# tpatten/squirrel_motion_planner

Hardware: AMD Instinct MI355X
Metric: collision-checked samples/sec + time-to-first-feasible-path, 8-DoF, 5 cm octomap (higher is better)
Workload: dtype f64

## Files before the change

### squirrel_motion_planner_amd/csrc/smp_kernels.hip

```cpp
#include <hip/hip_runtime.h>

#include <vector>

#include "smp_collide.h"
#include "smp_math.h"
#include "smp_plan.h"
#include "smp_types.h"

extern "C" __device__ __attribute__((const)) unsigned long long __ockl_wfred_min_u64(unsigned long long);
extern "C" __device__ __attribute__((const)) unsigned long long __ockl_wfred_max_u64(unsigned long long);

namespace smp {

constexpr int CHECK_CT = 32;

__shared__ RobotDev g_rb;
__shared__ MapCfg g_mc;
__shared__ WideStash g_wk;

__device__ __forceinline__ void stage_model(const RobotDev* rb, const MapCfg* mc, RobotDev* rbl, MapCfg* mcl) {
  static_assert(sizeof(RobotDev) % 8 == 0 && sizeof(MapCfg) % 4 == 0, "staging granularity");
  for (int i = threadIdx.x; i < (int)(sizeof(RobotDev) / 8); i += BLOCK)
    reinterpret_cast<uint64_t*>(rbl)[i] = reinterpret_cast<const uint64_t*>(rb)[i];
  for (int i = threadIdx.x; i < (int)(sizeof(MapCfg) / 4); i += BLOCK)
// ... 122 lines not shown
    }
  __syncthreads();
  for (int wd = 0; wd < (nsph + 31) / 32; ++wd) {
    uint32_t m = cand[wd];
    while (m) {
      const int s = wd * 32 + __builtin_ctz(m);
      m &= m - 1;
      const int c = rb->sph_clink[s];
      if (lm[c]) continue;
      const bool hit = wave_sphere_map(sc, wc[s], rb->sph_r[s], lane);
      __syncthreads();
      if (hit && lane == 0) lm[c] = 1;
      __syncthreads();
    }
  }
  for (int c = lane; c < rb->n_clink; c += 64) link_map[c] = (uint8_t)lm[c];
  for (int p = lane; p < rb->n_pairs; p += 64) {
    const int a = rb->pair_a[p], b = rb->pair_b[p];
    bool hit = false;
    if (rb->cl_prim[a] >= 0 || rb->cl_prim[b] >= 0) {
      const int pr = rb->cl_prim[a] >= 0 ? rb->cl_prim[a] : rb->cl_prim[b], sl = rb->cl_prim[a] >= 0 ? b : a;
      for (int s = rb->cl_sph0[sl]; s < rb->cl_sph0[sl] + rb->cl_nsph[sl] && !hit; ++s)
        hit = sphere_prim(rb->prim_type[pr], &rb->prim_h[pr * 3], pwl[pr], wc[s], rb->sph_r[s]);
      pair_self[p] = hit ? 1 : 0;
      continue;
    }
    for (int sa = rb->cl_sph0[a]; sa < rb->cl_sph0[a] + rb->cl_nsph[a] && !hit; ++sa)
      for (int sb = rb->cl_sph0[b]; sb < rb->cl_sph0[b] + rb->cl_nsph[b]; ++sb) {
        const double rs = rb->sph_r[sa] + rb->sph_r[sb];
        const double ex = wc[sa][0] - wc[sb][0], ey = wc[sa][1] - wc[sb][1], ez = wc[sa][2] - wc[sb][2];
        if (ex * ex + ey * ey + ez * ez <= rs * rs) { hit = true; break; }
      }
    pair_self[p] = hit ? 1 : 0;
  }
}

void launch_collisions(hipStream_t st, const RobotDev* rb, SceneDev sc, const MapCfg* mc, const double* q, int map,
                       uint8_t* link_map, uint8_t* pair_self) {
  hipLaunchKernelGGL(collisions_kernel, dim3(1), dim3(64), 0, st, rb, sc, mc, q, map, link_map, pair_self);
}

__global__ void sincos_kernel(const double* x, int n, double* s, double* c) {
  int i = blockIdx.x * blockDim.x + threadIdx.x;
  if (i < n) psincos(x[i], s + i, c + i);
}

__global__ void u01_kernel(unsigned long long seed, unsigned query, const uint32_t* ctr, int n, double* out) {
  int i = blockIdx.x * blockDim.x + threadIdx.x;
  if (i < n) out[i] = u01(seed, query, ctr[4 * i], ctr[4 * i + 1], ctr[4 * i + 2], ctr[4 * i + 3]);
}

__global__ void __launch_bounds__(128) fk_kernel(const RobotDev* __restrict__ rb, const double* q, int n, double* frames, double* eez) {
  int i = blockIdx.x * blockDim.x + threadIdx.x;
  if (i >= n) return;
  double qq[NJ];
  for (int j = 0; j < NJ; ++j) qq[j] = q[i * NJ + j];
  Frame B[MAX_BODY];
  body_frames(rb, qq, B);
  for (int b = 0; b < rb->n_body; ++b) {
    for (int k = 0; k < 9; ++k) frames[((size_t)i * rb->n_body + b) * 12 + k] = B[b].R[k];
    for (int k = 0; k < 3; ++k) frames[((size_t)i * rb->n_body + b) * 12 + 9 + k] = B[b].p[k];
  }
  eez[i] = ee_z(rb, qq);
}

__global__ void sqrt_div_kernel(const double* a, const double* b, int n, double* sq, double* dv) {
  int i = blockIdx.x * blockDim.x + threadIdx.x;
  if (i < n) { sq[i] = sqrt(a[i]); dv[i] = a[i] / b[i]; }
}

constexpr int SCAN_K = 20;
constexpr int NEAR_BINS = 256;
constexpr int NEAR_BUF = 128;
#ifndef SMP_NEAR_NBK
#define SMP_NEAR_NBK 16
#endif
constexpr int NEAR_NBK = SMP_NEAR_NBK;
struct ScanLds {
  union {
    struct {
      unsigned long long wlk[BLOCK / 64][SCAN_K], whk[BLOCK / 64][SCAN_K];
      int wli[BLOCK / 64][SCAN_K], whi[BLOCK / 64][SCAN_K];
    };
    struct {
      alignas(16) unsigned hist[NEAR_BINS];
      unsigned long long ck[2][NEAR_BUF];
      int ci[2][NEAR_BUF];
    };
  };
  unsigned long long hmin[BLOCK / 64], hmax[BLOCK / 64];
  int hcnt[2], hblo, hbhi, fast;
  int wtot[BLOCK / 64];
  unsigned long long blo, bhi;
  unsigned long long lk[SCAN_K], hk[SCAN_K];
  int li[SCAN_K], hi[SCAN_K];
  int cnt, take;
  unsigned long long wk[BLOCK / 64];
  int wi[BLOCK / 64];
};
constexpr int MERGE_LS = SCAN_K | 1;
struct MergeLds {
  unsigned kl[2][SCAN_PNEAR][MERGE_LS], kh[2][SCAN_PNEAR][MERGE_LS];
  int id[2][SCAN_PNEAR][MERGE_LS];
  int len[SCAN_P], cnt[SCAN_P], done[SCAN_P], bad[SCAN_P];
  unsigned hv[SCAN_P][3];
  unsigned hn[SCAN_PNEAR][3];
  unsigned long long nk[SCAN_P];
  int ni[SCAN_P];
  int ndone, go[2], steal;
};
__device__ __forceinline__ unsigned long long merge_key(const MergeLds& M, int s, int w, int e) {
  return (unsigned long long)M.kh[s][w][e] << 32 | M.kl[s][w][e];
}
struct JobLds {
#ifdef SMP_NO_SCAN_UNION
  ScanLds scan;
  WideLds T;
#else
  union {
    ScanLds scan;
    WideLds T;
  };
#endif
  double tq[TILE_CT_MAX][NJ];
  double start[MAXE][NJ], step[MAXE][NJ];
  unsigned words[JOB_WORDS];
  uint8_t rmask[JOB_TILES];
  uint8_t rdone[JOB_TILES];
  int emap[MAXE];
  int first[MAXE];
  int E, np1, nslots, ntiles, ct, self, map, seq, steal, hidx, left;
  int skip, sfv, tskip;
  int tgrp[TILE_CT_MAX], tord[TILE_CT_MAX];
  unsigned long long tprof[4];
  int go[2];
};
struct SmpLds {
  double q[64][NJ];
  int ok[64];
  int win;
};
struct SamplerLds {
  QState S;
  SmpLds W;
  double out[NJ];
  long long next;
  int ver, go[2];
};
#ifndef SMP_PLAN_CT
#define SMP_PLAN_CT 8
#endif
constexpr int PLAN_CT = SMP_PLAN_CT;
constexpr int PATCH_K = 32;
struct PlanLds {
  QState S;
  union {
    struct {
      TileLds<PLAN_CT> T;
      double tq[PLAN_CT][NJ];
    } tile;
    JobLds job;
    double seg[MAXE][MAX_PTS][3];
    SmpLds smp;
    SamplerLds smpl;
  } u;
  union {
    struct {
      struct {
        unsigned long long wlk[BLOCK / 64][MAX_NEAR], whk[BLOCK / 64][MAX_NEAR];
        int wli[BLOCK / 64][MAX_NEAR], whi[BLOCK / 64][MAX_NEAR];
        int wtot[BLOCK / 64];
      } nr;
      struct {
        alignas(16) unsigned hist[NEAR_BINS];
        unsigned long long ck[2][NEAR_BUF];
        int ci[2][NEAR_BUF];
        unsigned long long wmin[BLOCK / 64], wmax[BLOCK / 64];
        int wtot[BLOCK / 64];
        int cnt[2], blo, bhi, fast;
      } nh;
    };
    struct {
      ScanLds s;
      MergeLds m;
    } sc;
  };
  double eg_start[MAXE][NJ], eg_target[MAXE][NJ], eg_step[MAXE][NJ], eg_end[MAXE][NJ];
  double eg_base[MAXE][3], eg_cost[MAXE][3];
  double eg_acc[MAXE][3];
  int eg_first[MAXE], eg_need[MAXE], eg_near[MAXE], eg_ptr[MAXE];
  int rw_par[MAXE], rw_next;
  double rw_cost[MAXE][3];
  int tile_e[PLAN_CT], tile_i[PLAN_CT], tile_n;
  int count_slot;
  int job_seq;
  int in_job;
  int go_end;
  int smp_ver, smp_have_sol, smp_hit;
  int smp_pub;
  int spec, spec_nn;
  long long spec_cnt;
  double smp_cbest[3];
  int nk;
  unsigned long long near_blo, near_bhi;
  int lo_i[MAX_NEAR], hi_i[MAX_NEAR];
  double lo_c[MAX_NEAR], hi_c[MAX_NEAR];
  int n_lo, n_hi;
  NodeRef nn, xn, xc, cur, g;
  double xr[NJ], ext[NJ], ox[NJ];
  double en_start[NJ], en_target[NJ];
  int ext_nn, ext_bp, flag, found, nn_id, cnt;
  int reached;
  int n_via, nn_t, tree_expand;
  NodeRef sel;
  double sel_start[NJ], sel_target[NJ];
  double csp[3], best_nv;
  double sol[3];
  double wd[BLOCK / 64];
  unsigned long long wk[BLOCK / 64];
  int wi[BLOCK / 64];
  long long wcount[BLOCK / 64];
  ScoutRec sr;
  PreRec prer;
  int prer_ok;
#ifdef SMP_TRACE
  int trole;
  unsigned tn;
  long long tit;
#endif
  int sp_on, sp_stage, sp_go[2];
  double fnn_d;
  int fnn_id;
#ifdef SMP_SCAN_PROF
  unsigned long long spc_t;
#endif
  int sc_same[MAX_SCOUTS];
  unsigned sc_seen, sc_dead;
  int asked[SCOUT_SLOTS];
  int asked_conn[SCOUT_SLOTS];
  int asked_pre[SCOUT_SLOTS];
  int conn_rec;
  int two_scouts;
  unsigned sc_mod;
  unsigned rw_at0;
  int n_at0;
  int sc_t, sc_rerun;
  int sc_stale_f;
  double sc_hq[MAXE][NJ], sc_hc[MAXE];
  int sc_hp[MAXE];
  int rb_go[2];
  long long sc_k;
  int eg_hit[MAXE];
  int eg_rec[MAXE];
  int rec_grp;
  int rec_all, ev_job;
  double pc_q[2][PATCH_K][NJ];
};

__shared__ PlanLds g_L;

struct Ctx {
  SceneDev sc;
  QueryDev Q;
};

#ifdef SMP_TRACE
#ifndef SMP_TRACE_IT0
#define SMP_TRACE_IT0 3000
#endif
#ifndef SMP_TRACE_IT1
#define SMP_TRACE_IT1 3040
#endif
constexpr unsigned TLOG_CAP = 1u << 18, TLOG_ROLE = TLOG_CAP / 4;
__device__ unsigned long long g_tlog[TLOG_CAP];
__device__ unsigned g_tlog_n[4];
#define TR()                                                                                                  \
  if (threadIdx.x == 0 && g_L.tit >= SMP_TRACE_IT0 && g_L.tit < SMP_TRACE_IT1 && g_L.tn < TLOG_ROLE) {        \
    g_tlog[g_L.trole * TLOG_ROLE + g_L.tn] =                                                                   \
        ((unsigned long long)g_L.trole << 62) | ((unsigned long long)((g_L.tit - SMP_TRACE_IT0) & 0xff) << 54) | \
        ((unsigned long long)(__LINE__ & 0x3fff) << 40) | (wall_clock64() & 0xffffffffffull);                  \
    g_tlog_n[g_L.trole] = ++g_L.tn;                                                                            \
  }
#else
#define TR()
#endif

enum { P_SAMPLE, P_NN, P_EXPAND, P_NEAR, P_CHOOSE, P_REWIRE, P_CONNECT, P_TILES, P_NTILES, P_COSTS, P_VIA, P_NVIA,
       P_TFK, P_TCHAIN, P_TCENTRE, P_TTEST, P_XEXPAND, P_XCHOOSE, P_XREWIRE, P_XCONNECT };
#ifdef SMP_NOCLK
__device__ __forceinline__ unsigned long long pclk() { return 0; }
#else
__device__ __forceinline__ unsigned long long pclk() { return wall_clock64(); }
#endif
#define PROF_BEGIN() unsigned long long _pt = threadIdx.x == 0 ? pclk() : 0
#ifdef SMP_DETAIL_PROF
#define DETAIL_BEGIN(v) const unsigned long long v = threadIdx.x == 0 ? wall_clock64() : 0
#define DETAIL_END(v, k) if (threadIdx.x == 0) g_L.S.prof[k] += wall_clock64() - v
#else
#define DETAIL_BEGIN(v)
#define DETAIL_END(v, k)
#endif
#define PROF_END(k) if (threadIdx.x == 0) { g_L.S.prof[k] += pclk() - _pt; }

__device__ __forceinline__ int lane_id() { return threadIdx.x & 63; }
__device__ __forceinline__ int uni(int v) { return __builtin_amdgcn_readfirstlane(v); }
__device__ __forceinline__ int wave_id() { return threadIdx.x >> 6; }
typedef const double __attribute__((address_space(1)))* gcdptr;
__device__ __forceinline__ gcdptr uni_gptr(const double* p) {
  const unsigned long long v = reinterpret_cast<unsigned long long>(p);
  const unsigned lo = __builtin_amdgcn_readfirstlane((int)(unsigned)v);
  const unsigned hi = __builtin_amdgcn_readfirstlane((int)(unsigned)(v >> 32));
  return (gcdptr)(((unsigned long long)hi << 32) | lo);
}

__device__ __forceinline__ gcdptr uni_g(gcdptr p) {
  const unsigned long long v = reinterpret_cast<unsigned long long>(p);
  const unsigned lo = __builtin_amdgcn_readfirstlane((int)(unsigned)v);
  const unsigned hi = __builtin_amdgcn_readfirstlane((int)(unsigned)(v >> 32));
  return (gcdptr)(((unsigned long long)hi << 32) | lo);
}
__device__ __forceinline__ void tree_cols(gcdptr tq, int cap, gcdptr* c) {
#pragma unroll
  for (int j = 0; j < NJ; ++j) c[j] = uni_g(tq + (size_t)j * (unsigned)cap);
}
__device__ __forceinline__ bool wave_group_live(int first, int end) {
  return __builtin_amdgcn_readfirstlane((int)(first < end)) != 0;
}
__device__ __forceinline__ double ld_col(gcdptr col, unsigned i) {
  return *(gcdptr)((const char __attribute__((address_space(1)))*)col + i * 8u);
}
typedef const float __attribute__((address_space(1)))* gcfptr;
__device__ __forceinline__ float ld_col(gcfptr col, unsigned i) {
  return *(gcfptr)((const char __attribute__((address_space(1)))*)col + i * 4u);
}
template <int K, int NPT, typename P, typename T>
__device__ __forceinline__ void load_round_k(T (*a)[NJ], const P* cols, int b0, int i1, const T* fill) {
#pragma unroll
  for (int u = 0; u < NPT; ++u) {
    if (u < K) {
      const unsigned ii = (unsigned)min(b0 + u * BLOCK, i1 - 1);
#pragma unroll
      for (int j = 0; j < NJ; ++j) a[u][j] = ld_col(cols[j], ii);
    } else {
#pragma unroll
      for (int j = 0; j < NJ; ++j) a[u][j] = fill[j];
    }
  }
}
template <int NPT, typename P, typename T>
__device__ __forceinline__ void load_round(T (*a)[NJ], const P* cols, int b0, int i1, const T* fill) {
  static_assert(NPT == 8, "rounds of 8 nodes per thread");
  const int first = b0 - lane_id();
  const int nl = uni(min(NPT, (i1 - first + BLOCK - 1) / BLOCK));
  if (nl > 4) load_round_k<8, NPT>(a, cols, b0, i1, fill);
  else if (nl > 2) load_round_k<4, NPT>(a, cols, b0, i1, fill);
  else if (nl > 1) load_round_k<2, NPT>(a, cols, b0, i1, fill);
  else load_round_k<1, NPT>(a, cols, b0, i1, fill);
}

__device__ __forceinline__ void st_tree(double* p, double v) { *p = v; }
__device__ __forceinline__ void st_tree(int* p, int v) { *p = v; }
__device__ __forceinline__ void st_tree(float* p, float v) { *p = v; }
__device__ __forceinline__ void st_coord(const TreeDev& T, int cap, int j, int i, double v) {
  st_tree(&T.q[(size_t)j * cap + i], v);
  st_tree(&T.qf[(size_t)j * cap + i], (float)v);
}
__device__ __forceinline__ int xcc_id() { return __builtin_amdgcn_s_getreg((3 << 11) | 20); }
__device__ __forceinline__ bool same8(const double* a, const double* b) {
  bool s = true;
#pragma unroll
  for (int j = 0; j < NJ; ++j) s &= __double_as_longlong(a[j]) == __double_as_longlong(b[j]);
  return s;
}

#ifdef SMP_BOUNDS
__device__ int g_dbg[8];
#define BCHK(id, lim, line, t)                                                                          \
  if ((unsigned)(id) >= (unsigned)(lim)) {                                                             \
    if (atomicCAS(&g_dbg[0], 0, (line)) == 0) { g_dbg[1] = (id); g_dbg[2] = blockIdx.x; g_dbg[3] = (t); g_dbg[4] = (lim); } \
    id = 0;                                                                                            \
  }
#else
#define BCHK(id, lim, line, t)
#endif
#define load_node(C, t, id, o) load_node_at(C, t, id, o, __LINE__)
__device__ __forceinline__ void load_node_at(const Ctx& C, int t, int id, NodeRef* o, int line) {
  const TreeDev& T = C.Q.tr[t];
  const int cap = g_L.S.cap;
  BCHK(id, cap, line, t);
  (void)line;
  for (int j = 0; j < NJ; ++j) o->q[j] = T.q[(size_t)j * cap + id];
  for (int k = 0; k < 3; ++k) o->c[k] = T.cost[(size_t)k * cap + id];
  o->id = id;
  o->parent = T.parent[id];
}

__device__ void insert_node(const Ctx& C, int t, const double* e_start, const double* e_target, const NodeRef& x) {
  QState& S = g_L.S;
  int i = S.n[t];
  if (i >= S.cap || x.id != i) { S.status = -7; S.phase = 2; return; }
  const TreeDev& T = C.Q.tr[t];
  int cap = S.cap;
  for (int j = 0; j < NJ; ++j) {
    st_coord(T, cap, j, i, x.q[j]);
    T.e_start[(size_t)j * cap + i] = e_start[j];
    T.e_target[(size_t)j * cap + i] = e_target[j];
    g_L.pc_q[t][i & (PATCH_K - 1)][j] = x.q[j];
  }
  for (int k = 0; k < 3; ++k) st_tree(&T.cost[(size_t)k * cap + i], x.c[k]);
  st_tree(&T.parent[i], x.parent);
  T.first_child[i] = -1;
  int p = x.parent;
// ... 1245 lines not shown
      if (threadIdx.x == 0) { g_L.n_lo = take_c; g_L.n_hi = take_c; }
      __syncthreads();
      NEAR_COUNT(27);
      continue;
    }
    const double cmin = __longlong_as_double((long long)kmin), cmax = __longlong_as_double((long long)kmax);
    const double scale = cmax > cmin ? (NEAR_BINS * (1.0 - 1e-9)) / (cmax - cmin) : 0.0;
    unsigned bins[NEAR_NBK / 4] = {};
#pragma unroll
    for (int b = 0; b < NEAR_NBK; ++b)
      if (nmask >> b & 1) {
        const int bin = near_bin(key[b], cmin, scale);
        bins[b >> 2] |= (unsigned)bin << (8 * (b & 3));
        atomicAdd(&g_L.nh.hist[bin], 1u);
      }
    __syncthreads();
    NEAR_CLOCK(2);
    if (wave == 0) {
      const uint4 hv = reinterpret_cast<const uint4*>(g_L.nh.hist)[lane];
      const unsigned h0 = hv.x, h1 = hv.y, h2 = hv.z, h3 = hv.w;
      const int inc = wave_incl_scan(h0 + h1 + h2 + h3);
      const int c3 = inc, c2 = c3 - (int)h3, c1 = c2 - (int)h2, c0b = c1 - (int)h1;
      const int e0 = c0b - (int)h0;
      const int flo = c0b >= take_c ? 0 : c1 >= take_c ? 1 : c2 >= take_c ? 2 : c3 >= take_c ? 3 : 4;
      const int Llo = __builtin_ctzll(__ballot(flo < 4));
      const int blo = 4 * Llo + __builtin_amdgcn_readlane(flo, Llo);
      const int cnt_lo = __builtin_amdgcn_readlane(flo == 0 ? c0b : flo == 1 ? c1 : flo == 2 ? c2 : c3, Llo);
      const int lim = tot - take_c;
      const int fhi = c2 <= lim ? 3 : c1 <= lim ? 2 : c0b <= lim ? 1 : e0 <= lim ? 0 : -1;
      const int Lhi = 63 - __builtin_clzll(__ballot(fhi >= 0));
      const int fh = __builtin_amdgcn_readlane(fhi, Lhi);
      const int bhi = 4 * Lhi + fh;
      const int cnt_hi = tot - __builtin_amdgcn_readlane(fhi == 3 ? c2 : fhi == 2 ? c1 : fhi == 1 ? c0b : e0, Lhi);
      if (lane == 0) {
        g_L.nh.blo = blo;
        g_L.nh.bhi = bhi;
        g_L.nh.fast = cnt_lo + prev_lo <= NEAR_BUF && cnt_hi + prev_hi <= NEAR_BUF;
        g_L.nh.cnt[0] = prev_lo;
        g_L.nh.cnt[1] = prev_hi;
      }
    }
    if (threadIdx.x < prev_lo) {
      g_L.nh.ck[0][threadIdx.x] = (unsigned long long)__double_as_longlong(g_L.lo_c[threadIdx.x]);
      g_L.nh.ci[0][threadIdx.x] = g_L.lo_i[threadIdx.x];
    }
    if (threadIdx.x >= 64 && threadIdx.x < 64 + prev_hi) {
      g_L.nh.ck[1][threadIdx.x - 64] = (unsigned long long)__double_as_longlong(g_L.hi_c[threadIdx.x - 64]);
      g_L.nh.ci[1][threadIdx.x - 64] = g_L.hi_i[threadIdx.x - 64];
    }
    __syncthreads();
    NEAR_CLOCK(3);
    if (!uni(g_L.nh.fast)) {
      NEAR_COUNT(26);
      __syncthreads();
      near_set_stream<K, NN>(C, t, q, excl);
      return;
    }
    const int blo = g_L.nh.blo, bhi = g_L.nh.bhi;
#pragma unroll
    for (int g = 0; g < NEAR_NBK; ++g) {
      if (c0 + g * BLOCK + wave * 64 < n) {
        const bool nr = nmask >> g & 1;
        const int bin = bins[g >> 2] >> (8 * (g & 3)) & 255;
        const int i = c0 + g * BLOCK + wave * 64 + lane;
        if (nr && bin <= blo) {
          const int slot = atomicAdd(&g_L.nh.cnt[0], 1);
          g_L.nh.ck[0][slot] = key[g];
          g_L.nh.ci[0][slot] = i;
        }
        if (nr && bin >= bhi) {
          const int slot = atomicAdd(&g_L.nh.cnt[1], 1);
          g_L.nh.ck[1][slot] = key[g];
          g_L.nh.ci[1][slot] = i;
        }
      }
    }
    __syncthreads();
    NEAR_CLOCK(4);
    const int take = min(K, tot_all + tot);
    {
      const int e = threadIdx.x >= 256;
      const int idx = threadIdx.x & 255;
      const int m = g_L.nh.cnt[e];
      const int L = m <= 64 ? 4 : 2;
      const int c = L == 4 ? idx >> 2 : idx >> 1, sl = idx & (L - 1);
      int rank = 0;
      unsigned long long ck = 0;
      int ci = 0;
      if (c < m) {
        ck = g_L.nh.ck[e][c];
        ci = g_L.nh.ci[e][c];
        for (int j = sl; j < m; j += L) {
          const unsigned long long ok = g_L.nh.ck[e][j];
          const int oi = g_L.nh.ci[e][j];
          rank += e == 0 ? ki_less(ok, oi, ck, ci) : ki_less(ck, ci, ok, oi);
        }
      }
      rank += quad_xor1(rank);
      if (L == 4) rank += quad_xor2(rank);
      if (c < m && sl == 0 && rank < take) {
        if (e == 0) { g_L.lo_c[rank] = __longlong_as_double((long long)ck); g_L.lo_i[rank] = ci; }
        else { g_L.hi_c[take - 1 - rank] = __longlong_as_double((long long)ck); g_L.hi_i[take - 1 - rank] = ci; }
      }
    }
    tot_all += tot;
    if (threadIdx.x == 0) { g_L.n_lo = take; g_L.n_hi = take; }
    __syncthreads();
    NEAR_CLOCK(5);
    NEAR_COUNT(27);
  }
  if (threadIdx.x == 0) { g_L.nk = tot_all; g_L.S.near_nodes += n; }
  __syncthreads();
  if (NN) fnn_reduce(nb, nbi);
  TR();
}

template <int K, bool NN>
__device__ __noinline__ void near_set_scan(const Ctx& C, int t, const double* q, int excl) {
  [[clang::always_inline]] near_set<K, NN>(C, t, q, excl, false);
}

__device__ __forceinline__ unsigned rev_mask(const RobotDev* rb) {
  unsigned m = 0;
#pragma unroll
  for (int j = 0; j < NJ; ++j) m |= (rb->rev[j] != 0 ? 1u : 0u) << j;
  return m;
}

__device__ __forceinline__ double readlane_d(double v, int l) {
  const unsigned long long b = (unsigned long long)__double_as_longlong(v);
  const unsigned lo = (unsigned)__builtin_amdgcn_readlane((int)(unsigned)b, l);
  const unsigned hi = (unsigned)__builtin_amdgcn_readlane((int)(unsigned)(b >> 32), l);
  return __longlong_as_double((long long)(((unsigned long long)hi << 32) | lo));
}

__device__ __forceinline__ void seg_terms(unsigned rm, const double* st, const double* stp, int s, double& t, double& r,
                                          double& p) {
  t = 0.0; r = 0.0; p = 0.0;
#pragma unroll
  for (int j = 0; j < NJ; ++j) {
    const double a = st[j] + s * stp[j];
    const double b = st[j] + (s + 1) * stp[j];
    const double d = (b - a) * (b - a);
    t += d * 1.0;
    const bool rv = (rm >> j) & 1u;
    r += rv ? d : 0.0;
    p += rv ? 0.0 : d;
  }
}
__device__ __forceinline__ void seg_norms(unsigned rm, const double* st, const double* stp, int s, double& t, double& r,
                                          double& p) {
  seg_terms(rm, st, stp, s, t, r, p);
  t = sqrt(t); r = sqrt(r); p = sqrt(p);
}

__device__ void edge_costs(const Ctx& C, int E) {
  TR();
  PROF_BEGIN();
  const int np = g_L.S.n_pts;
  const RobotDev* rb = (&g_rb);
  if (threadIdx.x < E * NJ) {
    int e = threadIdx.x / NJ, j = threadIdx.x - e * NJ;
    double st = (g_L.eg_target[e][j] - g_L.eg_start[e][j]) / double(np);
    g_L.eg_step[e][j] = st;
    g_L.eg_end[e][j] = g_L.eg_start[e][j] + np * st;
  }
  __syncthreads();
  const unsigned rm = rev_mask(rb);
  for (int it = threadIdx.x; it < E * np; it += BLOCK) {
    const int e = it / np, s = it - e * np;
    double st[NJ], stp[NJ], t, r, p;
#pragma unroll
    for (int j = 0; j < NJ; ++j) { st[j] = g_L.eg_start[e][j]; stp[j] = g_L.eg_step[e][j]; }
    seg_norms(rm, st, stp, s, t, r, p);
    g_L.u.seg[e][s][0] = t;
    g_L.u.seg[e][s][1] = r;
    g_L.u.seg[e][s][2] = p;
  }
  __syncthreads();
  if (threadIdx.x < E * 3) {
    int e = threadIdx.x / 3, k = threadIdx.x - e * 3;
    double sg[MAX_PTS];
#pragma unroll
    for (int s = 0; s < MAX_PTS; ++s) sg[s] = g_L.u.seg[e][s][k];
    double acc = 0.0;
#pragma unroll
    for (int s = 0; s < MAX_PTS; ++s)
      if (s < np) acc += sg[s];
    g_L.eg_acc[e][k] = acc;
    g_L.eg_cost[e][k] = g_L.eg_base[e][k] + acc;
  }
  __syncthreads();
  PROF_END(P_COSTS);
  TR();
}

__device__ void edge_costs_acc(int E, const double (*acc)[3]) {
  const int np = g_L.S.n_pts;
  if (threadIdx.x < E * NJ) {
    const int e = threadIdx.x / NJ, j = threadIdx.x - e * NJ;
    const double st = (g_L.eg_target[e][j] - g_L.eg_start[e][j]) / double(np);
    g_L.eg_step[e][j] = st;
    g_L.eg_end[e][j] = g_L.eg_start[e][j] + np * st;
  } else if (threadIdx.x >= 256 && threadIdx.x < 256 + E * 3) {
    const int i = threadIdx.x - 256, e = i / 3, k = i - e * 3;
    const double a = acc[e][k];
    g_L.eg_acc[e][k] = a;
    g_L.eg_cost[e][k] = g_L.eg_base[e][k] + a;
  }
  __syncthreads();
}

#define TRACE(C, slot, v) \
  if ((C).Q.trace) __hip_atomic_store(&(C).Q.trace[slot], (int)(v), __ATOMIC_RELAXED, __HIP_MEMORY_SCOPE_SYSTEM)
__device__ __forceinline__ void st_agent(int* p, int v) { __hip_atomic_store(p, v, __ATOMIC_RELAXED, __HIP_MEMORY_SCOPE_AGENT); }
__device__ __forceinline__ void st_agent(unsigned long long* p, unsigned long long v) {
  __hip_atomic_store(p, v, __ATOMIC_RELAXED, __HIP_MEMORY_SCOPE_AGENT);
}
__device__ __forceinline__ int ld_agent(const int* p) { return __hip_atomic_load(p, __ATOMIC_RELAXED, __HIP_MEMORY_SCOPE_AGENT); }
__device__ __forceinline__ unsigned long long ld_agent(const unsigned long long* p) {
  return __hip_atomic_load(p, __ATOMIC_RELAXED, __HIP_MEMORY_SCOPE_AGENT);
}
__device__ __forceinline__ unsigned ld_agent(const unsigned* p) {
  return __hip_atomic_load(p, __ATOMIC_RELAXED, __HIP_MEMORY_SCOPE_AGENT);
}
__device__ __forceinline__ void drain() { asm volatile("s_waitcnt vmcnt(0)" ::: "memory"); }

__device__ __forceinline__ unsigned long long granule(int seq, unsigned w) {
  return ((unsigned long long)(unsigned)seq << 32) | w;
}

__device__ __forceinline__ bool job_tile_skip(const Ctx& C, JobLds& J, int t, int seq) {
  const JobBoard* jb = C.Q.jb;
  const int np1 = uni(J.np1), ne = uni(J.E), ct = uni(J.ct);
  for (int u = threadIdx.x; u < t; u += BLOCK) {
    if (!J.rdone[u]) {
      const unsigned long long v = ld_agent(&jb->res[u]);
      if ((int)(v >> 32) == seq) { J.rmask[u] = (unsigned)v; J.rdone[u] = 1; }
    }
  }
  if (threadIdx.x < ne) J.first[threadIdx.x] = np1;
  __syncthreads();
  for (int u = threadIdx.x; u < t; u += BLOCK) {
    if (!J.rdone[u]) continue;
    unsigned m = J.rmask[u];
    while (m) {
      const int sl = u * ct + __builtin_ctz(m), k = sl / np1;
      m &= m - 1;
      atomicMin(&J.first[k], sl - k * np1);
    }
  }
  __syncthreads();
  if (threadIdx.x < 64) {
    const int lane = threadIdx.x;
    bool fr = false;
    if (J.sfv && lane < ne && (lane + 1) * np1 <= t * ct && J.first[lane] >= np1) {
      fr = true;
      for (int u = (lane * np1) / ct; u <= ((lane + 1) * np1 - 1) / ct; ++u)
        if (!J.rdone[u]) { fr = false; break; }
    }
    const unsigned long long fb = __ballot(fr);
    const int ff = fb ? __builtin_ctzll(fb) : (1 << 30);
    const int base = t * ct, nc = min(ct, J.nslots - base);
    bool live = false;
    if (lane < nc) {
      const int sl = base + lane, k = sl / np1, i = sl - k * np1;
      live = k <= ff && i <= J.first[k];
      J.tgrp[lane] = k;
      J.tord[lane] = live ? i : (1 << 30);
    }
    const unsigned long long lb = __ballot(live);
    if (lane == 0) J.tskip = lb == 0;
  }
  __syncthreads();
  return uni(J.tskip) != 0;
}

struct DirectJob {
  unsigned hdr;
  int ne;
};
__device__ __forceinline__ unsigned job_tile_mask(const Ctx& C, const WideConst& K, JobLds& J, int t,
                                                  unsigned long long* prof = nullptr, int seq = -1,
                                                  const DirectJob* direct = nullptr, bool sync_after = true) {
  int ct, nc, self, map;
  bool sk = false;
  if (direct) {
    const unsigned hdr = direct->hdr;
    const int ne = direct->ne;
    const int np1 = (int)((hdr >> 8) & 255);
    ct = 1 << ((hdr >> 21) & 3);
    const int base = t * ct;
    nc = min(ct, ne * np1 - base);
    self = (int)((hdr >> 16) & 1);
    map = (int)((hdr >> 17) & 1);
    const int c = (int)(threadIdx.x >> 6) / (NWAVE / ct), j = threadIdx.x & 63;
    if (c < nc && j < NJ) {
      const int sl = base + c, k = sl / np1, i = sl - k * np1, wi = 1 + 32 * k + 2 * j;
      const double qs = __hiloint2double((int)J.words[wi + 1], (int)J.words[wi]);
      const double qd = __hiloint2double((int)J.words[wi + 2 * NJ + 1], (int)J.words[wi + 2 * NJ]);
      J.tq[c][j] = qs + i * qd;
    }
    wave_sync();
  } else {
    ct = uni(J.ct);
    const int base = t * ct;
// ... 1062 lines not shown
      if (threadIdx.x < E && g_L.eg_hit[threadIdx.x] >= 0) g_L.eg_first[threadIdx.x] = g_L.eg_hit[threadIdx.x];
      __syncthreads();
    }
    TR();
    return;
  }
  if (threadIdx.x < E) { g_L.eg_first[threadIdx.x] = np1; g_L.eg_ptr[threadIdx.x] = 0; }
  sc_early_send(C, early, epar, E, true);
  __syncthreads();
  for (;;) {
    if (threadIdx.x < 64) {
      const int e = threadIdx.x;
      const bool live = e < E && g_L.eg_need[e] && g_L.eg_first[e] >= np1;
      const int ptr = e < E ? g_L.eg_ptr[e] : np1;
      bool stop = false;
      if (stop_first_valid) {
        const unsigned long long m = __ballot(live);
        if (m) stop = __shfl(ptr, __builtin_ctzll(m)) >= np1;
      }
      const int rem = (live && ptr < np1) ? np1 - ptr : 0;
      int inc = rem;
      for (int off = 1; off < 32; off <<= 1) {
        int v = __shfl_up(inc, off);
        if (e >= off) inc += v;
      }
      const int start = inc - rem;
      const int take = stop ? 0 : max(0, min(rem, PLAN_CT - start));
      for (int i = 0; i < take; ++i) { g_L.tile_e[start + i] = e; g_L.tile_i[start + i] = ptr + i; }
      if (e < E) g_L.eg_ptr[e] = ptr + take;
      const int total = __shfl(inc, 31);
      if (e == 0) g_L.tile_n = stop ? 0 : min(PLAN_CT, total);
    }
    __syncthreads();
    const int nc = uni(g_L.tile_n);
    if (nc == 0) break;
    if (threadIdx.x < nc * NJ) {
      int c = threadIdx.x / NJ, j = threadIdx.x - c * NJ;
      int e = g_L.tile_e[c];
      g_L.u.tile.tq[c][j] = g_L.eg_start[e][j] + g_L.tile_i[c] * g_L.eg_step[e][j];
    }
    __syncthreads();
    PROF_BEGIN();
    local_tile(C, nc);
    PROF_END(P_TILES);
    if (threadIdx.x == 0) {
      g_L.S.prof[pslot] += pclk() - _pt;
      g_L.S.prof[P_NTILES]++;
      g_L.S.prof[pslot + 8] += nc;
    }
  }
  __syncthreads();
  overlap_work(C, ov, ovt);
}

__device__ void overlap_work(const Ctx& C, int ov, int t) {
  ov = uni(ov);
  t = uni(t);
  if (ov == OV_NONE) {
    if (threadIdx.x == 0) g_L.spec = OV_NONE;
    __syncthreads();
    return;
  }
  const long long c0 = ov == OV_NN ? g_L.S.nn_nodes : g_L.S.near_nodes;
  __syncthreads();
  if (ov == OV_NEAR_EXPAND) near_set<20>(C, t, g_L.eg_end[0], g_L.S.n[t], true);
  else if (ov == OV_NEAR_XN) near_set<20>(C, t, g_L.xn.q, g_L.xn.id);
  else {
    const int id = nearest(C, t, g_L.xn.q);
    if (threadIdx.x == 0) g_L.spec_nn = id;
  }
  if (threadIdx.x == 0) {
    long long& cnt = ov == OV_NN ? g_L.S.nn_nodes : g_L.S.near_nodes;
    g_L.spec_cnt = cnt - c0;
    cnt = c0;
    g_L.spec = ov;
  }
  __syncthreads();
}

__device__ __forceinline__ void count_edge(int first) {
  int np1 = g_L.S.n_pts + 1;
  g_L.S.prof[g_L.count_slot] += first >= np1 ? np1 : first + 1;
  if (first >= np1) { g_L.S.checked += np1; g_L.S.valid += np1; }
  else { g_L.S.checked += first + 1; g_L.S.valid += first; }
}

__device__ int count_edges(int E, bool stop_first) {
  if (threadIdx.x < 64) {
    const int e = threadIdx.x, np1 = g_L.S.n_pts + 1;
    const bool need = e < E && g_L.eg_need[e];
    const int f = need ? g_L.eg_first[e] : 0;
    const unsigned long long mfree = __ballot(need && f >= np1);
    const int ev = (stop_first && mfree) ? __builtin_ctzll(mfree) : 64;
    int chk = 0, val = 0;
    if (need && e <= ev) { chk = f >= np1 ? np1 : f + 1; val = f >= np1 ? np1 : f; }
    chk = __ockl_wfred_add_i32(chk); val = __ockl_wfred_add_i32(val);
    if (e == 0) {
      g_L.S.prof[g_L.count_slot] += chk;
      g_L.S.checked += chk;
      g_L.S.valid += val;
      g_L.found = ev < 64 ? ev : -1;
    }
  }
  __syncthreads();
  return uni(g_L.found);
}

__device__ __forceinline__ bool step_towards_m(unsigned rm, const double* nn, double* x, double f) {
  double ed[NJ], srev = 0.0, spr = 0.0;
#pragma unroll
  for (int j = 0; j < NJ; ++j) {
    const bool rv = (rm >> j) & 1u;
    ed[j] = x[j] - nn[j];
    const double d = ed[j] * ed[j];
    srev += rv ? d : 0.0;
    spr += rv ? 0.0 : d;
  }
  const double lrev = sqrt(srev), lpr = sqrt(spr);
  const bool rev_done = lrev < 0.001, pr_done = lpr < 0.001;
  double ext[NJ];
  srev = 0.0; spr = 0.0;
#pragma unroll
  for (int j = 0; j < NJ; ++j) {
    const bool rv = (rm >> j) & 1u;
    const bool done = rv ? rev_done : pr_done;
    const double c = f * (ed[j] / (rv ? lrev : lpr));
    ext[j] = done ? 0.0 : nn[j] + c;
    const double cc = done ? 0.0 : c * c;
    srev += rv ? cc : 0.0;
    spr += rv ? 0.0 : cc;
  }
  const double elp = spr == 0.0 ? 1000.0 : sqrt(spr);
  const double elr = srev == 0.0 ? 1000.0 : sqrt(srev);
  const bool tr = elr < lrev, tp = elp < lpr;
#pragma unroll
  for (int j = 0; j < NJ; ++j) {
    const bool rv = (rm >> j) & 1u;
    if (rv ? tr : tp) x[j] = ext[j];
  }
  return !(tr || tp);
}
__device__ bool step_towards(const RobotDev* rb, const double* nn, double* x, double f) {
  return step_towards_m(rev_mask(rb), nn, x, f);
}

__device__ __forceinline__ bool step_towards_w(unsigned rm, const double* nn, double* x, double f, int lane, double nn_l,
                                               double& x_l) {
  double ed[NJ], srev = 0.0, spr = 0.0;
#pragma unroll
  for (int j = 0; j < NJ; ++j) {
    const bool rv = (rm >> j) & 1u;
    ed[j] = x[j] - nn[j];
    const double d = ed[j] * ed[j];
    srev += rv ? d : 0.0;
    spr += rv ? 0.0 : d;
  }
  const double l2 = sqrt((lane & 1) ? spr : srev);
  const double lrev = readlane_d(l2, 0), lpr = readlane_d(l2, 1);
  const bool rev_done = lrev < 0.001, pr_done = lpr < 0.001;
  const bool rvl = (rm >> (lane & 7)) & 1u;
  const double ql = (x_l - nn_l) / (rvl ? lrev : lpr);
  double ext[NJ];
  srev = 0.0; spr = 0.0;
#pragma unroll
  for (int j = 0; j < NJ; ++j) {
    const bool rv = (rm >> j) & 1u;
    const bool done = rv ? rev_done : pr_done;
    const double c = f * readlane_d(ql, j);
    ext[j] = done ? 0.0 : nn[j] + c;
    const double cc = done ? 0.0 : c * c;
    srev += rv ? cc : 0.0;
    spr += rv ? 0.0 : cc;
  }
  const double e2 = sqrt((lane & 1) ? spr : srev);
  const double elr = srev == 0.0 ? 1000.0 : readlane_d(e2, 0);
  const double elp = spr == 0.0 ? 1000.0 : readlane_d(e2, 1);
  const bool tr = elr < lrev, tp = elp < lpr;
#pragma unroll
  for (int j = 0; j < NJ; ++j) {
    const bool rv = (rm >> j) & 1u;
    if (rv ? tr : tp) x[j] = ext[j];
  }
  if (rvl ? tr : tp) x_l = (rvl ? rev_done : pr_done) ? 0.0 : nn_l + f * ql;
  return !(tr || tp);
}

__device__ __noinline__ void via_chain_w(const Ctx& C, const double* target) {
  const int lane = lane_id(), s = lane & 31;
  const int np = g_L.S.n_pts, via_cap = g_L.S.via_cap;
  const double f = g_L.S.step;
  double cur[NJ], cc[3], tg[NJ], ox[NJ], stp[NJ], end[NJ], acc[3], cost[3];
  int cid = g_L.cur.id, cpar = g_L.cur.parent;
#pragma unroll
  for (int j = 0; j < NJ; ++j) { cur[j] = g_L.cur.q[j]; tg[j] = target[j]; }
#pragma unroll
  for (int k = 0; k < 3; ++k) cc[k] = g_L.cur.c[k];
  int nn_t = g_L.nn_t, n_via = g_L.n_via, nsteps = 0;
  const unsigned rm = rev_mask(&g_rb);
  double cur_l = g_L.cur.q[lane & 7], ox_l;
  const double tg_l = target[lane & 7];
  static_assert(NJ == 8, "lane copies of the joints");
#ifdef SMP_VIA_PROF
  unsigned long long _v0 = wall_clock64(), _v1;
#define VIA_CLK(k) { _v1 = wall_clock64(); if (lane == 0) g_L.S.prof[k] += _v1 - _v0; _v0 = _v1; }
#else
#define VIA_CLK(k)
#endif
  VIA_CLK(31);
  bool reached, overflow = false;
  double lst[NJ], lcc[3];
  for (;;) {
    ++nsteps;
#pragma unroll
    for (int j = 0; j < NJ; ++j) ox[j] = tg[j];
    ox_l = tg_l;
    reached = step_towards_w(rm, cur, ox, f, lane, cur_l, ox_l);
    const double ql = (ox_l - cur_l) / double(np);
#pragma unroll
    for (int j = 0; j < NJ; ++j) {
      stp[j] = readlane_d(ql, j);
      end[j] = cur[j] + np * stp[j];
    }
    VIA_CLK(28);
    if (np <= 21) {
      const int k = lane / 21, sg = lane - 21 * k;
      double t, r, p;
      seg_terms(rm, cur, stp, sg, t, r, p);
      const double v = sqrt(k == 0 ? t : k == 1 ? r : p);
      if (sg < np && k < 3) g_L.u.seg[0][sg][k] = v;
    } else {
      double t, r, p;
      seg_norms(rm, cur, stp, s, t, r, p);
      if (lane < np) { g_L.u.seg[0][lane][0] = t; g_L.u.seg[0][lane][1] = r; g_L.u.seg[0][lane][2] = p; }
    }
    VIA_CLK(29);
    double al = 0.0;
    if (lane < 3) {
      double sg[MAX_PTS];
#pragma unroll
      for (int i = 0; i < MAX_PTS; ++i) sg[i] = g_L.u.seg[0][i][lane];
#pragma unroll
      for (int i = 0; i < MAX_PTS; ++i)
        if (i < np) al += sg[i];
    }
#pragma unroll
    for (int k = 0; k < 3; ++k) acc[k] = readlane_d(al, k);
    VIA_CLK(30);
#pragma unroll
    for (int k = 0; k < 3; ++k) cost[k] = cc[k] + acc[k];
#pragma unroll
    for (int j = 0; j < NJ; ++j) lst[j] = cur[j];
#pragma unroll
    for (int k = 0; k < 3; ++k) lcc[k] = cc[k];
    if (reached) break;
    const int id = nn_t++;
    if (n_via >= via_cap) { overflow = true; reached = true; break; }
    if (lane == 0) {
      ViaNode& v = C.Q.via[n_via];
#pragma unroll
      for (int j = 0; j < NJ; ++j) { v.q[j] = end[j]; v.e_start[j] = cur[j]; v.e_target[j] = ox[j]; }
#pragma unroll
      for (int k = 0; k < 3; ++k) v.c[k] = cost[k];
      v.id = id;
      v.parent = cid;
    }
    ++n_via;
    cpar = cid;
    cid = id;
    cur_l = cur_l + np * ql;
#pragma unroll
    for (int j = 0; j < NJ; ++j) cur[j] = end[j];
#pragma unroll
    for (int k = 0; k < 3; ++k) cc[k] = cost[k];
  }
#undef VIA_CLK
  if (lane == 0) {
    QState& S = g_L.S;
    S.prof[P_NVIA] += nsteps;
    if (overflow) { S.status = -7; S.phase = 2; }
    else {
      NodeRef& g = g_L.sel;
#pragma unroll
      for (int j = 0; j < NJ; ++j) { g.q[j] = end[j]; g_L.sel_start[j] = cur[j]; g_L.sel_target[j] = ox[j]; }
#pragma unroll
      for (int k = 0; k < 3; ++k) g.c[k] = cost[k];
      g.id = nn_t;
      g.parent = cid;
    }
    g_L.reached = 1;
    g_L.nn_t = nn_t;
    g_L.n_via = n_via;
#pragma unroll
    for (int j = 0; j < NJ; ++j) {
      g_L.cur.q[j] = cur[j];
      g_L.ox[j] = ox[j];
      g_L.eg_start[0][j] = lst[j];
      g_L.eg_target[0][j] = ox[j];
      g_L.eg_step[0][j] = stp[j];
      g_L.eg_end[0][j] = end[j];
    }
#pragma unroll
    for (int k = 0; k < 3; ++k) {
      g_L.cur.c[k] = cc[k];
      g_L.eg_base[0][k] = lcc[k];
      g_L.eg_acc[0][k] = acc[k];
      g_L.eg_cost[0][k] = cost[k];
    }
    g_L.cur.id = cid;
    g_L.cur.parent = cpar;
  }
}
__device__ void via_chain(const Ctx& C, const double* target) {
  TR();
  PROF_BEGIN();
  if (threadIdx.x < 64) via_chain_w(C, target);
  __syncthreads();
  PROF_END(P_VIA);
  TR();
}

__device__ void insert_via(const Ctx& C, int t, const ViaNode* rec = nullptr, int rec_x = 0) {
  TR();
  DETAIL_BEGIN(_di);
  const int nv = uni(g_L.n_via);
  if (nv > 0) {
    QState& S = g_L.S;
    const TreeDev& T = C.Q.tr[t];
    const int n0 = uni(S.n[t]), cap = uni(S.cap);
    if (n0 + nv > cap) {
      if (threadIdx.x == 0) { S.status = -7; S.phase = 2; }
    } else {
      for (int k = threadIdx.x; k < nv; k += BLOCK) {
        const ViaNode& w = rec ? rec[k] : C.Q.via[k];
        auto ldd = [&](const double* p) {
          return rec ? __longlong_as_double((long long)ld_agent(reinterpret_cast<const unsigned long long*>(p))) : *p;
        };
        int wid = rec ? ld_agent(&w.id) : w.id, wpar = rec ? ld_agent(&w.parent) : w.parent;
        if (rec) {
          const int off = n0 - rec_x;
          if (wid >= rec_x) wid += off;
          if (wpar >= rec_x) wpar += off;
        }
        const int i = n0 + k;
        if (wid != i || (k > 0 && wpar != i - 1)) S.status = -7;
        for (int j = 0; j < NJ; ++j) {
          const double qj = ldd(&w.q[j]);
          st_coord(T, cap, j, i, qj);
          g_L.pc_q[t][i & (PATCH_K - 1)][j] = qj;
          T.e_start[(size_t)j * cap + i] = ldd(&w.e_start[j]);
          T.e_target[(size_t)j * cap + i] = ldd(&w.e_target[j]);
        }
        for (int c = 0; c < 3; ++c) st_tree(&T.cost[(size_t)c * cap + i], ldd(&w.c[c]));
        st_tree(&T.parent[i], wpar);
        T.first_child[i] = k + 1 < nv ? i + 1 : -1;
        T.prev_sib[i] = -1;
        if (k > 0) {
          T.next_sib[i] = -1;
        } else {
          const int p = wpar, f = T.first_child[p];
          T.next_sib[i] = f;
          if (f >= 0) T.prev_sib[f] = i;
          T.first_child[p] = i;
        }
      }
      if (threadIdx.x == 0) {
        S.n[t] = n0 + nv;
        S.edges[t] += nv;
      }
    }
  }
  __syncthreads();
  if (threadIdx.x == 0) {
    if (g_L.S.status == -7) g_L.S.phase = 2;
    g_L.n_via = 0;
  }
  DETAIL_END(_di, 31);
  __syncthreads();
  TR();
}

#ifdef SMP_RING_CHECK
__device__ unsigned long long g_ringchk[64];
__device__ unsigned long long g_ringdbg[SMP_RING][16];
extern "C" void smp_ringchk_dump() {
  unsigned long long v[64];
  if (hipMemcpyFromSymbol(v, HIP_SYMBOL(g_ringchk), sizeof(v)) == hipSuccess) {
    double d[64];
    __builtin_memcpy(d, v, sizeof(d));
    std::fprintf(stderr, "[smp] ring check: uniform(it) %llu, it-1 %llu, it+1 %llu, other %llu; first mismatch it %llu\n",
                 v[0], v[1], v[2], v[3], v[4]);
    std::fprintf(stderr, "[smp]   ring  :");
    for (int j = 0; j < 8; ++j) std::fprintf(stderr, " %.17g", d[24 + j]);
    std::fprintf(stderr, "\n[smp]   leader:");
    for (int j = 0; j < 8; ++j) std::fprintf(stderr, " %.17g", d[32 + j]);
    std::fprintf(stderr, "\n[smp]   sampler h0 %.17g Crev0 %.17g Crev7 %.17g ctr0 %.17g qmin2 %.17g qmax2 %.17g rev %llx\n",
                 d[40], d[41], d[42], d[43], d[44], d[45], v[46]);
    std::fprintf(stderr, "[smp]   leader  h0 %.17g Crev0 %.17g Crev7 %.17g ctr0 %.17g qmin2 %.17g qmax2 %.17g rev %llx\n",
                 d[48], d[49], d[50], d[51], d[52], d[53], v[54]);
  }
}
#endif
__device__ __forceinline__ void rand_conf_lane(const QState& S, uint32_t it, uint32_t outer, uint32_t inner, double* q) {
  const RobotDev* rb = (&g_rb);
  bool env0 = S.env_x[0] == 0.0 && S.env_x[1] == 0.0 && S.env_y[0] == 0.0 && S.env_y[1] == 0.0;
  double u[NJ];
#pragma unroll
  for (int p = 0; p < NJ / 2; ++p) u01_pair(S.seed, S.query, it, outer, inner, p, &u[2 * p], &u[2 * p + 1]);
#pragma unroll
  for (int j = 0; j < NJ; ++j) {
    double lo = rb->q_min[j], hi = rb->q_max[j];
    if (!env0 && j == 0) { lo = S.env_x[0]; hi = S.env_x[1]; }
    if (!env0 && j == 1) { lo = S.env_y[0]; hi = S.env_y[1]; }
    q[j] = u[j] * (hi - lo) + lo;
  }
}

__device__ __forceinline__ int sample_uniform(const QState& S, uint32_t it, SmpLds& W, double* out) {
  if (wave_id() == 0) {
    int st = -1;
    for (uint32_t base = 0; base < (1u << 24); base += 64) {
      double q[NJ];
      rand_conf_lane(S, it, 0, base + lane_id(), q);
      bool ok = 0.0 <= ee_z((&g_rb), q);
      unsigned long long m = __ballot(ok);
      if (m) {
        int w = __ffsll((long long)m) - 1;
        if (lane_id() == w) for (int j = 0; j < NJ; ++j) out[j] = q[j];
        st = 0;
        break;
      }
    }
    if (lane_id() == 0) W.win = st;
  }
  __syncthreads();
  return uni(W.win);
}

__device__ __forceinline__ int sample_ellipse(const QState& S, uint32_t it, SmpLds& W, double* out) {
  const RobotDev* rb = (&g_rb);
  const bool env0 = S.env_x[0] == 0.0 && S.env_x[1] == 0.0 && S.env_y[0] == 0.0 && S.env_y[1] == 0.0;
  const int lane = lane_id();
  constexpr int SE_OUT = 32;
  for (uint32_t base = 0;; base += SE_OUT) {
    if (base >= (1u << 20)) return -1;
    if (threadIdx.x < SE_OUT * 8) {
      const uint32_t b = base + (threadIdx.x >> 3), inner = threadIdx.x & 7;
      double q[NJ];
      rand_conf_lane(S, it, 1 + b, inner, q);
      const bool ok = 0.0 <= ee_z(rb, q);
      const unsigned long long m = __ballot(ok);
      const unsigned grp = (unsigned)(m >> (lane & ~7)) & 0xffu;
      const int first = grp ? __builtin_ctz(grp) : 8;
      if ((int)inner == first)
        for (int j = 0; j < NJ; ++j) W.q[threadIdx.x >> 3][j] = q[j];
      if (inner == 0) W.ok[threadIdx.x >> 3] = grp != 0;
    }
    __syncthreads();
    if (wave_id() == 0) {
      const uint32_t b = base + lane;
      double q[NJ];
      if (lane >= SE_OUT) {
        for (int j = 0; j < NJ; ++j) q[j] = 1.0;
      } else if (W.ok[lane]) {
        for (int j = 0; j < NJ; ++j) q[j] = W.q[lane][j];
      } else {
        for (uint32_t inner = 8; inner < (1u << 16); ++inner) {
          rand_conf_lane(S, it, 1 + b, inner, q);
          if (0.0 <= ee_z(rb, q)) break;
        }
// ... 2273 lines not shown
```

Baseline: 4.655 million.

## Batch via-chain steps and spread segment-cost work across all waves

The via chain used to run one step at a time on a single wavefront, computing segment norms, summing and writing each ViaNode serially. Now one wave computes up to 16 step endpoints into LDS. All waves then compute the per-segment costs in parallel, the costs are combined with an ordered prefix sum, and the ViaNodes are written one 8-byte word per thread. This is meant to cut the serial per-step latency, at the price of extra block-wide syncs per batch. Some accumulations also become FMAs with 0/1 masks, and the summation order is kept so f64 results stay deterministic.

```diff
diff --git a/squirrel_motion_planner_amd/csrc/smp_kernels.hip b/squirrel_motion_planner_amd/csrc/smp_kernels.hip
--- a/squirrel_motion_planner_amd/csrc/smp_kernels.hip
+++ b/squirrel_motion_planner_amd/csrc/smp_kernels.hip
@@ -298,6 +298,17 @@
 #endif
 constexpr int PLAN_CT = SMP_PLAN_CT;
 constexpr int PATCH_K = 32;
+constexpr int VIA_B = 16;
+struct ViaRow { double cur[NJ], ox[NJ], stp[NJ], end[NJ]; };
+struct ViaLds {
+  double seg[BLOCK / 64][MAX_PTS][3];
+  ViaRow row[VIA_B];
+  double acc[VIA_B][3];
+  int n, fin;
+};
+constexpr int VIA_WORDS = sizeof(ViaNode) / 8;
+static_assert(sizeof(ViaNode) == 8 * (3 * NJ + 3 + 1), "ViaNode as 8-byte words: q, c, e_start, e_target, {id, parent}");
+static_assert(VIA_B * VIA_WORDS <= BLOCK, "one ViaNode word per thread");
 struct PlanLds {
   QState S;
   union {
@@ -307,6 +318,7 @@
     } tile;
     JobLds job;
     double seg[MAXE][MAX_PTS][3];
+    ViaLds via;
     SmpLds smp;
     SamplerLds smpl;
   } u;
@@ -404,6 +416,7 @@
 };
 
 __shared__ PlanLds g_L;
+static_assert(sizeof(ViaLds) <= sizeof(g_L.u.seg), "a via chain's batch lies within the union's edge rows");
 
 struct Ctx {
   SceneDev sc;
@@ -1955,6 +1968,17 @@
                                           double& p) {
   seg_terms(rm, st, stp, s, t, r, p);
   t = sqrt(t); r = sqrt(r); p = sqrt(p);
+}
+
+template <int N>
+__device__ __forceinline__ double ordered_sum(const double (*seg)[3], int k) {
+  double t[N];
+#pragma unroll
+  for (int i = 0; i < N; ++i) t[i] = seg[i][k];
+  double acc = 0.0;
+#pragma unroll
+  for (int i = 0; i < N; ++i) acc += t[i];
+  return acc;
 }
 
 __device__ void edge_costs(const Ctx& C, int E) {
@@ -3323,8 +3347,8 @@
     const bool rv = (rm >> j) & 1u;
     ed[j] = x[j] - nn[j];
     const double d = ed[j] * ed[j];
-    srev += rv ? d : 0.0;
-    spr += rv ? 0.0 : d;
+    srev = __builtin_fma(d, rv ? 1.0 : 0.0, srev);
+    spr = __builtin_fma(d, rv ? 0.0 : 1.0, spr);
   }
   const double l2 = sqrt((lane & 1) ? spr : srev);
   const double lrev = readlane_d(l2, 0), lpr = readlane_d(l2, 1);
@@ -3340,8 +3364,8 @@
     const double c = f * readlane_d(ql, j);
     ext[j] = done ? 0.0 : nn[j] + c;
     const double cc = done ? 0.0 : c * c;
-    srev += rv ? cc : 0.0;
-    spr += rv ? 0.0 : cc;
+    srev = __builtin_fma(cc, rv ? 1.0 : 0.0, srev);
+    spr = __builtin_fma(cc, rv ? 0.0 : 1.0, spr);
   }
   const double e2 = sqrt((lane & 1) ? spr : srev);
   const double elr = srev == 0.0 ? 1000.0 : readlane_d(e2, 0);
@@ -3356,136 +3380,168 @@
   return !(tr || tp);
 }
 
-__device__ __noinline__ void via_chain_w(const Ctx& C, const double* target) {
-  const int lane = lane_id(), s = lane & 31;
-  const int np = g_L.S.n_pts, via_cap = g_L.S.via_cap;
+__device__ __noinline__ void via_steps_w(const double* target) {
+  ViaLds& V = g_L.u.via;
+  const int lane = lane_id();
+  const int np = g_L.S.n_pts, room = g_L.S.via_cap - g_L.n_via;
   const double f = g_L.S.step;
-  double cur[NJ], cc[3], tg[NJ], ox[NJ], stp[NJ], end[NJ], acc[3], cost[3];
-  int cid = g_L.cur.id, cpar = g_L.cur.parent;
+  double cur[NJ], tg[NJ], ox[NJ];
 #pragma unroll
   for (int j = 0; j < NJ; ++j) { cur[j] = g_L.cur.q[j]; tg[j] = target[j]; }
-#pragma unroll
-  for (int k = 0; k < 3; ++k) cc[k] = g_L.cur.c[k];
-  int nn_t = g_L.nn_t, n_via = g_L.n_via, nsteps = 0;
   const unsigned rm = rev_mask(&g_rb);
   double cur_l = g_L.cur.q[lane & 7], ox_l;
   const double tg_l = target[lane & 7];
   static_assert(NJ == 8, "lane copies of the joints");
+  int r = 0, fin = 0;
+  for (;;) {
+#pragma unroll
+    for (int j = 0; j < NJ; ++j) ox[j] = tg[j];
+    ox_l = tg_l;
+    const bool reached = uni(step_towards_w(rm, cur, ox, f, lane, cur_l, ox_l));
+    const double ql = (ox_l - cur_l) / double(np);
+    const double end_l = cur_l + np * ql;
+    if (lane < NJ) {
+      ViaRow& R = V.row[r];
+      R.cur[lane] = cur_l; R.ox[lane] = ox_l; R.stp[lane] = ql; R.end[lane] = end_l;
+    }
+    ++r;
+    if (reached) { fin = 1; break; }
+    if (r > room) { fin = 2; break; }
+    if (r == VIA_B) break;
+#pragma unroll
+    for (int j = 0; j < NJ; ++j) cur[j] = readlane_d(end_l, j);
+    cur_l = end_l;
+  }
+  if (lane == 0) { V.n = r; V.fin = fin; }
+}
+
+template <int R>
+__device__ __forceinline__ void via_prefix(const double* a, int n, int nv, double* vc, double& c, double& base, double& last) {
+  if constexpr (R < VIA_B) {
+    if (R < n) {
+      base = c;
+      last = a[R];
+      c = base + last;
+      if (R < nv) vc[R * VIA_WORDS] = c;
+      via_prefix<R + 1>(a, n, nv, vc, c, base, last);
+    }
+  }
+}
+
+__device__ __noinline__ bool via_costs(const Ctx& C) {
+  ViaLds& V = g_L.u.via;
+  QState& S = g_L.S;
 #ifdef SMP_VIA_PROF
-  unsigned long long _v0 = wall_clock64(), _v1;
-#define VIA_CLK(k) { _v1 = wall_clock64(); if (lane == 0) g_L.S.prof[k] += _v1 - _v0; _v0 = _v1; }
+  unsigned long long _v0 = threadIdx.x == 0 ? wall_clock64() : 0;
+#define VIA_CLK(k) if (threadIdx.x == 0) { const unsigned long long _v1 = wall_clock64(); S.prof[k] += _v1 - _v0; _v0 = _v1; }
 #else
 #define VIA_CLK(k)
 #endif
-  VIA_CLK(31);
-  bool reached, overflow = false;
-  double lst[NJ], lcc[3];
-  for (;;) {
-    ++nsteps;
-#pragma unroll
-    for (int j = 0; j < NJ; ++j) ox[j] = tg[j];
-    ox_l = tg_l;
-    reached = step_towards_w(rm, cur, ox, f, lane, cur_l, ox_l);
-    const double ql = (ox_l - cur_l) / double(np);
-#pragma unroll
-    for (int j = 0; j < NJ; ++j) {
-      stp[j] = readlane_d(ql, j);
-      end[j] = cur[j] + np * stp[j];
-    }
-    VIA_CLK(28);
+  const int n = uni(V.n), fin = uni(V.fin), np = uni(S.n_pts);
+  const int nv = fin ? n - 1 : n;
+  const int n_via0 = uni(g_L.n_via), nn_t0 = uni(g_L.nn_t), cid0 = uni(g_L.cur.id), cpar0 = uni(g_L.cur.parent);
+  const int w = wave_id(), lane = lane_id();
+  const unsigned rm = rev_mask(&g_rb);
+  for (int r = w; r < n; r += BLOCK / 64) {
+    double cur[NJ], stp[NJ];
+#pragma unroll
+    for (int j = 0; j < NJ; ++j) { cur[j] = V.row[r].cur[j]; stp[j] = V.row[r].stp[j]; }
     if (np <= 21) {
       const int k = lane / 21, sg = lane - 21 * k;
-      double t, r, p;
-      seg_terms(rm, cur, stp, sg, t, r, p);
-      const double v = sqrt(k == 0 ? t : k == 1 ? r : p);
-      if (sg < np && k < 3) g_L.u.seg[0][sg][k] = v;
+      double t, rr, p;
+      seg_terms(rm, cur, stp, sg, t, rr, p);
+      const double v = sqrt(k == 0 ? t : k == 1 ? rr : p);
+      if (k < 3) V.seg[w][sg][k] = sg < np ? v : 0.0;
+      if (lane < 3) V.acc[r][lane] = ordered_sum<21>(V.seg[w], lane);
     } else {
-      double t, r, p;
-      seg_norms(rm, cur, stp, s, t, r, p);
-      if (lane < np) { g_L.u.seg[0][lane][0] = t; g_L.u.seg[0][lane][1] = r; g_L.u.seg[0][lane][2] = p; }
-    }
-    VIA_CLK(29);
-    double al = 0.0;
-    if (lane < 3) {
-      double sg[MAX_PTS];
-#pragma unroll
-      for (int i = 0; i < MAX_PTS; ++i) sg[i] = g_L.u.seg[0][i][lane];
-#pragma unroll
-      for (int i = 0; i < MAX_PTS; ++i)
-        if (i < np) al += sg[i];
-    }
-#pragma unroll
-    for (int k = 0; k < 3; ++k) acc[k] = readlane_d(al, k);
-    VIA_CLK(30);
-#pragma unroll
-    for (int k = 0; k < 3; ++k) cost[k] = cc[k] + acc[k];
-#pragma unroll
-    for (int j = 0; j < NJ; ++j) lst[j] = cur[j];
-#pragma unroll
-    for (int k = 0; k < 3; ++k) lcc[k] = cc[k];
-    if (reached) break;
-    const int id = nn_t++;
-    if (n_via >= via_cap) { overflow = true; reached = true; break; }
-    if (lane == 0) {
-      ViaNode& v = C.Q.via[n_via];
-#pragma unroll
-      for (int j = 0; j < NJ; ++j) { v.q[j] = end[j]; v.e_start[j] = cur[j]; v.e_target[j] = ox[j]; }
-#pragma unroll
-      for (int k = 0; k < 3; ++k) v.c[k] = cost[k];
-      v.id = id;
-      v.parent = cid;
-    }
-    ++n_via;
-    cpar = cid;
-    cid = id;
-    cur_l = cur_l + np * ql;
-#pragma unroll
-    for (int j = 0; j < NJ; ++j) cur[j] = end[j];
-#pragma unroll
-    for (int k = 0; k < 3; ++k) cc[k] = cost[k];
-  }
+      double t, rr, p;
+      seg_norms(rm, cur, stp, lane & 31, t, rr, p);
+      const bool in = lane < np;
+      if (lane < MAX_PTS) { V.seg[w][lane][0] = in ? t : 0.0; V.seg[w][lane][1] = in ? rr : 0.0; V.seg[w][lane][2] = in ? p : 0.0; }
+      if (lane < 3) V.acc[r][lane] = ordered_sum<MAX_PTS>(V.seg[w], lane);
+    }
+  }
+  __syncthreads();
+  VIA_CLK(29);
+  {
+    const int r = threadIdx.x / VIA_WORDS, wd = threadIdx.x - r * VIA_WORDS;
+    if (r < nv && (wd < NJ || wd >= NJ + 3)) {
+      const unsigned long long* R = reinterpret_cast<const unsigned long long*>(&V.row[r]);
+      unsigned long long v;
+      if (wd < NJ) v = R[3 * NJ + wd];
+      else if (wd < 2 * NJ + 3) v = R[wd - (NJ + 3)];
+      else if (wd < 3 * NJ + 3) v = R[NJ + wd - (2 * NJ + 3)];
+      else {
+        const int id = nn_t0 + r, parent = r ? id - 1 : cid0;
+        v = (unsigned long long)(unsigned)id | ((unsigned long long)(unsigned)parent << 32);
+      }
+      reinterpret_cast<unsigned long long*>(&C.Q.via[n_via0 + r])[wd] = v;
+    }
+  }
+  if (threadIdx.x < 3) {
+    const int k = threadIdx.x;
+    double a[VIA_B];
+#pragma unroll
+    for (int i = 0; i < VIA_B; ++i) a[i] = V.acc[i][k];
+    double c = g_L.cur.c[k], base = c, last = 0.0;
+    via_prefix<0>(a, n, nv, &C.Q.via[n_via0].c[k], c, base, last);
+    if (fin) {
+      g_L.cur.c[k] = base;
+      g_L.eg_base[0][k] = base;
+      g_L.eg_acc[0][k] = last;
+      g_L.eg_cost[0][k] = c;
+      if (fin == 1) g_L.sel.c[k] = c;
+    } else {
+      g_L.cur.c[k] = c;
+    }
+  } else if (threadIdx.x >= 64 && threadIdx.x < 64 + NJ) {
+    const int j = threadIdx.x - 64;
+    const ViaRow& R = V.row[n - 1];
+    if (fin) {
+      const double st = R.cur[j], ox = R.ox[j], en = R.end[j];
+      g_L.cur.q[j] = st;
+      g_L.ox[j] = ox;
+      g_L.eg_start[0][j] = st;
+      g_L.eg_target[0][j] = ox;
+      g_L.eg_step[0][j] = R.stp[j];
+      g_L.eg_end[0][j] = en;
+      if (fin == 1) { g_L.sel.q[j] = en; g_L.sel_start[j] = st; g_L.sel_target[j] = ox; }
+    } else {
+      g_L.cur.q[j] = R.end[j];
+    }
+  } else if (threadIdx.x == 128) {
+    const int cid = nv ? nn_t0 + nv - 1 : cid0, nn_t = nn_t0 + nv + (fin == 2);
+    S.prof[P_NVIA] += n;
+    g_L.cur.id = cid;
+    g_L.cur.parent = nv == 0 ? cpar0 : nv == 1 ? cid0 : nn_t0 + nv - 2;
+    g_L.n_via = n_via0 + nv;
+    g_L.nn_t = nn_t;
+    if (fin) {
+      g_L.reached = 1;
+      if (fin == 2) { S.status = -7; S.phase = 2; }
+      else { g_L.sel.id = nn_t; g_L.sel.parent = cid; }
+    }
+  }
+  __syncthreads();
+  VIA_CLK(30);
 #undef VIA_CLK
-  if (lane == 0) {
-    QState& S = g_L.S;
-    S.prof[P_NVIA] += nsteps;
-    if (overflow) { S.status = -7; S.phase = 2; }
-    else {
-      NodeRef& g = g_L.sel;
-#pragma unroll
-      for (int j = 0; j < NJ; ++j) { g.q[j] = end[j]; g_L.sel_start[j] = cur[j]; g_L.sel_target[j] = ox[j]; }
-#pragma unroll
-      for (int k = 0; k < 3; ++k) g.c[k] = cost[k];
-      g.id = nn_t;
-      g.parent = cid;
-    }
-    g_L.reached = 1;
-    g_L.nn_t = nn_t;
-    g_L.n_via = n_via;
-#pragma unroll
-    for (int j = 0; j < NJ; ++j) {
-      g_L.cur.q[j] = cur[j];
-      g_L.ox[j] = ox[j];
-      g_L.eg_start[0][j] = lst[j];
-      g_L.eg_target[0][j] = ox[j];
-      g_L.eg_step[0][j] = stp[j];
-      g_L.eg_end[0][j] = end[j];
-    }
-#pragma unroll
-    for (int k = 0; k < 3; ++k) {
-      g_L.cur.c[k] = cc[k];
-      g_L.eg_base[0][k] = lcc[k];
-      g_L.eg_acc[0][k] = acc[k];
-      g_L.eg_cost[0][k] = cost[k];
-    }
-    g_L.cur.id = cid;
-    g_L.cur.parent = cpar;
-  }
-}
+  return fin != 0;
+}
+
 __device__ void via_chain(const Ctx& C, const double* target) {
   TR();
   PROF_BEGIN();
-  if (threadIdx.x < 64) via_chain_w(C, target);
-  __syncthreads();
+  for (;;) {
+#ifdef SMP_VIA_PROF
+    const unsigned long long _v0 = threadIdx.x == 0 ? wall_clock64() : 0;
+#endif
+    if (threadIdx.x < 64) via_steps_w(target);
+    __syncthreads();
+#ifdef SMP_VIA_PROF
+    if (threadIdx.x == 0) { g_L.S.prof[28] += wall_clock64() - _v0; g_L.S.prof[31] += 100; }
+#endif
+    if (via_costs(C)) break;
+  }
   PROF_END(P_VIA);
   TR();
 }
```

Result: faster. 4.847 million (median of 6 runs) (+4.1%).
